# cakarsubasi/02562_raytracer

Measured on AMD Instinct MI355X. Metric: Mrays/sec primary+shadow at 1920x1080; achieved HBM GB/s vs peak, higher is better.
Workload: dtype f32

## Files before the change

02562_raytracer_amd/__init__.py:

```python
from . import _ffi
from ._ffi import MODES, TRAVERSALS, RtError, lib
from .core import (BspTree, Bvh, Context, DeviceBuffer, Mesh, empty_mask_host, load_texture_rgba8, local_tiles,
                   make_uniform)
from .render_state import ASSETS, RenderState
from .camera import CameraController
from .scenes import Camera, SceneDescriptor, find_scene, get_scenes

__all__ = ["BspTree", "Bvh", "Camera", "CameraController", "Context", "DeviceBuffer", "Mesh", "RenderState", "RtError",
           "SceneDescriptor", "ASSETS", "MODES", "TRAVERSALS", "find_scene", "get_scenes", "lib", "local_tiles",
           "load_texture_rgba8",
           "make_uniform", "_ffi"]
```

02562_raytracer_amd/_ffi.py:

```python
import ctypes as C
import os

import numpy as np

PKG_DIR = os.path.dirname(os.path.abspath(__file__))
LIB_PATH = os.environ.get("RT_LIBRARY") or os.path.join(PKG_DIR, "lib02562rt.so")

RT_OK = 0
RT_E_INVALID = -1
RT_E_OOM = -2
RT_E_DEVICE = -3
RT_E_NOT_READY = -4
RT_E_IO = -5
RT_E_UNSUPPORTED = -6

(RT_MODE_W1E6, RT_MODE_W6E1, RT_MODE_PROJECT, RT_MODE_W7E3, RT_MODE_W9E1, RT_MODE_W8E1, RT_MODE_W8E2, RT_MODE_W8E3,
 RT_MODE_W9E2, RT_MODE_W6E2, RT_MODE_W7E1, RT_MODE_W7E2, RT_MODE_W6E3, RT_MODE_W9E3,
 RT_MODE_W5E2, RT_MODE_W5E3, RT_MODE_W5E4, RT_MODE_W5E5,
 RT_MODE_W2E1, RT_MODE_W2E2, RT_MODE_W2E3, RT_MODE_W2E4, RT_MODE_W2E5,
 RT_MODE_W3E1, RT_MODE_W3E2, RT_MODE_W3E3, RT_MODE_W3E4,
 RT_MODE_W1E2, RT_MODE_W1E3, RT_MODE_W1E4, RT_MODE_W1E5) = range(31)
RT_TRAVERSE_BSP, RT_TRAVERSE_BVH, RT_TRAVERSE_NONE = range(3)
RT_OPT_DETAIL_COUNTERS = 1
RT_OPT_WAVES_PER_CU = 2
RT_OPT_SHADE_THRESHOLD = 3
RT_OPT_SAMPLE_CHUNK = 4
RT_OPT_SAMPLE_BUDGET_MB = 5
RT_OPT_UNIT_ORDER = 6
RT_OPT_BSP_CULL = 9
RT_OPT_ASYNC_FOLD = 10
RT_OPT_EMPTY_PIXELS = 11
RT_BSP_CULL_OFF, RT_BSP_CULL_CERTIFIED, RT_BSP_CULL_FAST, RT_BSP_CULL_SILHOUETTE, RT_BSP_CULL_AUTO = range(5)
BSP_TREELET_BYTES = 96
RT_OPT_KERNEL_TIMING = 7
RT_COMM_ID_BYTES = 128

MODES = {"W1E6": RT_MODE_W1E6, "W6E1": RT_MODE_W6E1, "PROJECT": RT_MODE_PROJECT, "W7E3": RT_MODE_W7E3,
         "W9E1": RT_MODE_W9E1, "W8E1": RT_MODE_W8E1, "W8E2": RT_MODE_W8E2, "W8E3": RT_MODE_W8E3,
         "W9E2": RT_MODE_W9E2, "W6E2": RT_MODE_W6E2, "W7E1": RT_MODE_W7E1, "W7E2": RT_MODE_W7E2,
         "W6E3": RT_MODE_W6E3, "W9E3": RT_MODE_W9E3,
         "W5E2": RT_MODE_W5E2, "W5E3": RT_MODE_W5E3, "W5E4": RT_MODE_W5E4, "W5E5": RT_MODE_W5E5,
         "W2E1": RT_MODE_W2E1, "W2E2": RT_MODE_W2E2, "W2E3": RT_MODE_W2E3, "W2E4": RT_MODE_W2E4,
         "W2E5": RT_MODE_W2E5, "W3E1": RT_MODE_W3E1, "W3E2": RT_MODE_W3E2, "W3E3": RT_MODE_W3E3,
         "W3E4": RT_MODE_W3E4,
         "W1E2": RT_MODE_W1E2, "W1E3": RT_MODE_W1E3, "W1E4": RT_MODE_W1E4, "W1E5": RT_MODE_W1E5}
SWEEP_MODES = ("W5E2", "W5E3", "W5E4", "W5E5")
# ... 143 lines not shown
    "rt_comm_unique_id": (C.c_int, [vp]),
    "rt_comm_init": (C.c_int, [vp, C.c_uint32, C.c_uint32, vp]),
    "rt_comm_destroy": (C.c_int, [vp]),
    "rt_gather_tiles": (C.c_int, [vp, C.c_uint32, C.c_uint32, vp, vp, vp, vp]),
    "rt_trace_rays": (C.c_int, [vp, C.c_int, vp, vp, C.c_uint32, vp]),
    "rt_trace_batch": (C.c_int, [vp, C.c_int, vp, vp, C.c_uint32, vp]),
    "rt_set_ray_capture": (C.c_int, [vp, vp, vp, C.c_uint64]),
    "rt_ray_capture_count": (C.c_int, [vp, C.POINTER(C.c_uint64)]),
    "rt_last_counts": (C.c_int, [vp, C.POINTER(RayCounts)]),
    "rt_last_elided_shadows": (C.c_int, [vp, C.POINTER(C.c_uint64)]),
    "rt_last_elided_primaries": (C.c_int, [vp, C.POINTER(C.c_uint64)]),
    "rt_empty_pixels_in_use": (C.c_int, [vp, C.POINTER(C.c_uint64), f32p]),
    "rt_empty_mask_host": (C.c_int, [f32p, C.c_uint32, u32p, C.c_uint32, C.POINTER(Uniform), u32p,
                                     C.POINTER(C.c_uint64)]),
    "rt_download_empty_mask": (C.c_int, [vp, u32p, C.c_uint64]),
    "rt_selftest_math": (C.c_int, [vp, C.c_uint32, C.c_float, C.c_float, u32p]),
    "rt_mesh_load_obj": (C.c_int, [C.c_char_p, C.POINTER(vp)]),
    "rt_mesh_from_arrays": (C.c_int, [f32p, f32p, C.c_uint32, u32p, C.c_uint32, C.POINTER(Material), C.c_uint32,
                                      C.POINTER(vp)]),
    "rt_mesh_synth_bunny": (C.c_int, [C.c_uint32, C.c_uint32, C.POINTER(vp)]),
    "rt_mesh_synth_soup": (C.c_int, [C.c_uint32, C.c_uint32, C.POINTER(vp)]),
    "rt_mesh_synth_grid": (C.c_int, [vp, C.c_uint32, C.c_uint32, C.c_float, C.POINTER(vp)]),
    "rt_mesh_scale": (C.c_int, [vp, C.c_float]),
    "rt_mesh_view_get": (C.c_int, [vp, C.POINTER(MeshView)]),
    "rt_mesh_free": (None, [vp]),
    "rt_bsp_build": (C.c_int, [vp, C.c_uint32, C.c_uint32, C.c_int, C.POINTER(vp)]),
    "rt_bsp_view_get": (C.c_int, [vp, C.POINTER(BspView)]),
    "rt_bsp_free": (None, [vp]),
    "rt_bvh_build": (C.c_int, [vp, C.c_uint32, C.POINTER(vp)]),
    "rt_bvh_view_get": (C.c_int, [vp, C.POINTER(BvhView)]),
# ... 53 lines not shown
```

02562_raytracer_amd/core.py:

```python
import ctypes as C

import numpy as np

from . import _ffi as F


def _mats_from(ptr, n):
    if n == 0:
        return np.zeros((0, 16), dtype=np.float32)
    raw = np.ctypeslib.as_array(C.cast(ptr, F.f32p), shape=(n * 16,)).copy()
    return raw.reshape(n, 16)


class Mesh:

    def __init__(self, handle):
        self._h = C.c_void_p(handle) if not isinstance(handle, C.c_void_p) else handle

    def __del__(self):
        if getattr(self, "_h", None) and self._h.value and F._lib is not None:
            F._lib.rt_mesh_free(self._h)
            self._h = C.c_void_p(None)

    @property
# ... 436 lines not shown
        n = C.c_uint64()
        self._chk(F.lib().rt_last_elided_primaries(self._h, C.byref(n)))
        return n.value

    def empty_pixels_in_use(self):
        n = C.c_uint64()
        ms = C.c_float()
        self._chk(F.lib().rt_empty_pixels_in_use(self._h, C.byref(n), C.byref(ms)))
        return n.value, ms.value

    def download_empty_mask(self, width, height):
        words = np.zeros((width * height + 31) // 32, np.uint32)
        self._chk(F.lib().rt_download_empty_mask(self._h, F.as_u32p(words), words.size))
        return _mask_bits(words, width, height)

    def timer_start(self):
        self._chk(F.lib().rt_timer_start(self._h))

    def timer_stop(self):
        ms = C.c_float()
        self._chk(F.lib().rt_timer_stop(self._h, C.byref(ms)))
        return ms.value

    def frame_rgba8(self, accum_ptr, npix, out_ptr, mode=None):
        if mode is None:
            self._chk(F.lib().rt_frame_rgba8(self._h, C.c_void_p(accum_ptr), npix, C.c_void_p(out_ptr)))
        else:
            self._chk(F.lib().rt_frame_rgba8_mode(self._h, F.MODES.get(mode, mode), C.c_void_p(accum_ptr), npix,
                                                  C.c_void_p(out_ptr)))

# ... 32 lines not shown
def _mask_bits(words, width, height):
    bits = np.unpackbits(words.view(np.uint8), bitorder="little")[:width * height]
    return bits.reshape(height, width).astype(bool)


def empty_mask_host(mesh, uniform):
    V, _, I, _, _ = mesh.arrays()
    V = np.ascontiguousarray(V, np.float32)
    I = np.ascontiguousarray(I, np.uint32)
    W, H = int(uniform.resolution[0]), int(uniform.resolution[1])
    words = np.zeros((W * H + 31) // 32, np.uint32)
    n = C.c_uint64()
    F.check(F.lib().rt_empty_mask_host(F.as_f32p(V), V.shape[0], F.as_u32p(I), I.shape[0], C.byref(uniform),
                                       F.as_u32p(words), C.byref(n)))
    return _mask_bits(words, W, H)


def load_texture_rgba8(path):
    from PIL import Image
    with Image.open(path) as im:
        return np.asarray(im.convert("RGBA"), dtype=np.uint8).copy()


def synth_texture(size=64):
    y, x = np.meshgrid(np.arange(size, dtype=np.uint32), np.arange(size, dtype=np.uint32), indexing="ij")
    h = (x * np.uint32(73856093)) ^ (y * np.uint32(19349663))
    h = (h ^ (h >> np.uint32(13))) * np.uint32(0x5BD1E995)
    h = h ^ (h >> np.uint32(15))
    t = np.empty((size, size, 4), np.uint8)
    t[..., 0] = 40 + (h & np.uint32(63))
# ... 9 lines not shown
```

02562_raytracer_amd/csrc/rt_api.cpp:

```cpp
#include <dlfcn.h>
#include <hip/hip_runtime.h>
#include <rccl/rccl.h>
#include <stdint.h>
#include <string.h>

#include <algorithm>
#include <cfloat>
#include <cmath>
#include <string>
#include <thread>
#include <type_traits>
#include <vector>

#include "host_types.h"
#include "rt_internal.h"

namespace {

struct DevBuf {
    void* p = nullptr;
    size_t n = 0;
    ~DevBuf() { reset(); }
    void reset()
    {
// ... 108 lines not shown
    bool fold_pending = false;
    float* cap_rays = nullptr;
    uint32_t* cap_flags = nullptr;
    uint64_t cap_max = 0;
    DevBuf cap_count;
    rt_noise_state* noise = nullptr;
    DevBuf noise_sum;
    uint32_t empty_opt = 1;
    float mesh_scale = 0.0f;
    float empty_cam[16] = {};
    bool empty_has_cam = false, empty_valid = false, empty_tried = false;
    uint64_t empty_iters = 0, empty_flagged = 0;
    float empty_build_ms = 0.0f;
    hipEvent_t empty_ev[2] = {nullptr, nullptr};
    DevBuf empty_mask, empty_hit, empty_cnt, empty_big;
    DevBuf act_list, act_flags, act_offs, act_scan;
    uint32_t act_key[8] = {};
    uint32_t act_n = 0, act_flagged = 0;
    bool act_valid = false;
    bool empty_used = false;
    uint64_t elided_primaries = 0;
    ncclComm_t comm = nullptr;
    uint32_t comm_nranks = 0, comm_rank = 0;
    DevBuf gather_accum, gather_ids;
};

namespace {

int fail(rt_ctx* c, int code, const std::string& msg)
{
// ... 208 lines not shown
    case RT_OPT_ASYNC_FOLD:
        if (value < 0 || value > 1) return fail(c, RT_E_INVALID, "async fold must be 0 or 1");
        if (int r = set_dev(c)) return r;
        if (value && !c->fold_stream) {
            HIPCHK(c, hipStreamCreateWithFlags(&c->fold_stream, hipStreamNonBlocking));
            for (hipEvent_t* e : {&c->ev_path, &c->ev_enter, &c->ev_fold, &c->ev_free[0], &c->ev_free[1]})
                HIPCHK(c, hipEventCreateWithFlags(e, hipEventDisableTiming));
        }
        c->async_fold = value != 0;
        return RT_OK;
    case RT_OPT_EMPTY_PIXELS:
        if (value < 0 || value > 2)
            return fail(c, RT_E_INVALID, "empty pixels must be 0 (off), 1 (on) or 2 (on, built at the first render)");
        c->empty_opt = (uint32_t)value;
        return RT_OK;
    case RT_OPT_SAMPLE_BUDGET_MB:
        if (value < 1 || value > (1 << 20)) return fail(c, RT_E_INVALID, "sample budget must be in [1,2^20] MiB");
        c->sample_budget_mb = (uint64_t)value;
        return RT_OK;
    default:
        return fail(c, RT_E_INVALID, "unknown option");
    }
}

const char* rt_last_error(const rt_ctx* c) { return c ? c->err.c_str() : rthost::get_error(); }

int rt_device_alloc(rt_ctx* c, size_t bytes, void** dptr)
{
    if (!c || !dptr) return RT_E_INVALID;
    if (int r = set_dev(c)) return r;
// ... 814 lines not shown
        unsigned long long* area_d = c->empty_cnt.as<unsigned long long>();
        uint32_t* flagged_d = c->empty_cnt.as<uint32_t>() + 2;
        uint32_t* nbig_d = c->empty_cnt.as<uint32_t>() + 3;
        HIPCHK(c, c->empty_big.ensure((size_t)std::max<uint32_t>(c->ntris, 1u) * 4));
        if (rtk::launch_empty_area(c->pos.as<float4>(), c->idx.as<uint4>(), c->nverts, c->ntris, cam14, W, H,
                                   c->mesh_scale, area_d, c->empty_big.as<uint32_t>(), nbig_d, c->stream))
            return fail(c, RT_E_DEVICE, "empty-pixel mask: launch failed");
        unsigned long long area = 0;
        uint32_t nbig = 0;
        HIPCHK(c, hipMemcpyAsync(&area, area_d, 8, hipMemcpyDeviceToHost, c->stream));
        HIPCHK(c, hipMemcpyAsync(&nbig, nbig_d, 4, hipMemcpyDeviceToHost, c->stream));
        HIPCHK(c, hipStreamSynchronize(c->stream));
        if (area <= kEmptyBudgetPerPixel * npix) {
            HIPCHK(c, c->empty_hit.ensure(npix));
            HIPCHK(c, c->empty_mask.ensure((npix + 31) / 32 * 4));
            for (hipEvent_t& e : c->empty_ev)
                if (!e) HIPCHK(c, hipEventCreate(&e));
            HIPCHK(c, hipEventRecord(c->empty_ev[0], c->stream));
            if (rtk::launch_empty_mask(c->pos.as<float4>(), c->idx.as<uint4>(), c->nverts, c->ntris, cam14, W, H,
                                       c->mesh_scale, c->empty_big.as<uint32_t>(), std::min(nbig, c->ntris),
                                       c->empty_hit.as<uint8_t>(), c->empty_mask.as<uint32_t>(), flagged_d, c->stream))
                return fail(c, RT_E_DEVICE, "empty-pixel mask: launch failed");
            HIPCHK(c, hipEventRecord(c->empty_ev[1], c->stream));
            uint32_t flagged = 0;
            HIPCHK(c, hipMemcpyAsync(&flagged, flagged_d, 4, hipMemcpyDeviceToHost, c->stream));
            HIPCHK(c, hipStreamSynchronize(c->stream));
            HIPCHK(c, hipEventElapsedTime(&c->empty_build_ms, c->empty_ev[0], c->empty_ev[1]));
            c->empty_flagged = flagged;
            c->empty_valid = true;
            c->act_valid = false;
            if (!c->auto_cull) c->probe_n = 0;
        }
    }
    *use = c->empty_valid && c->empty_flagged > 0;
    return RT_OK;
}
// ... 112 lines not shown
    L.work_counter = c->work.as<uint32_t>();
    L.cap_rays = reinterpret_cast<float4*>(c->cap_rays);
    L.cap_flags = c->cap_flags;
    L.cap_count = c->cap_count.as<unsigned long long>();
    L.cap_max = c->cap_max;
    if (trav == RT_TRAVERSE_BVH) {
        const size_t need = rtk::bvh_deep_bytes(c->num_cus, c->waves_per_cu);
        if (c->bvh_deep.n < need) HIPCHK(c, c->bvh_deep.alloc(need));
        L.bvh_deep = c->bvh_deep.as<uint32_t>();
    }
    const bool sil = has_silhouette(c, mode, trav);
    S.bsp_cull_mode = cull_in_use(c, sil);
    L.shade_threshold = default_threshold(c, mode, trav, S.bsp_cull_mode);
    L.counters = c->counters.as<unsigned long long>();
    HIPCHK(c, hipMemsetAsync(c->counters.p, 0, 32 * sizeof(unsigned long long), c->stream));
    c->empty_used = false;
    c->elided_primaries = 0;
    if (L.nwork == 0 || (L.spp == 0 && (path || direct_prog))) {
        if (counts) return rt_last_counts(c, counts);
        return RT_OK;
    }
    if (path) {
        L.stride = L.tileset ? L.nwork * 64u : L.w * L.h;
        bool ep = false;
        if (empty_applies(c, mode, trav)) {
            if (int r = ensure_empty(c, L.cam, L.spp, &ep)) return r;
            if (ep)
                if (int r = ensure_active(c, L)) return r;
            if (ep) {
                c->empty_used = true;
                c->elided_primaries = (uint64_t)c->act_flagged * L.spp;
            }
        }
        const bool nothing_active = ep && L.nactive == 0;
        const uint32_t* emask = ep ? c->empty_mask.as<uint32_t>() : nullptr;
        const uint64_t per_it = (uint64_t)L.stride * sizeof(float4);
        const uint64_t budget = c->sample_budget_mb << 20;
        uint32_t pass_spp = (uint32_t)std::min<uint64_t>(L.spp, std::max<uint64_t>(1, budget / per_it));
        const uint64_t need = per_it * pass_spp;
        const bool async = c->async_fold && c->fold_stream;
        if (c->samples.n < need) HIPCHK(c, c->samples.alloc(need));
        if (async && c->samples2.n < need) HIPCHK(c, c->samples2.alloc(need));
        L.samples = c->samples.as<float4>();
        const bool autop = sil && c->bsp_cull == RT_BSP_CULL_AUTO && c->hcam_valid && !c->detail && !nothing_active;
        if (autop)
            if (int r = probe_begin(c)) return r;
// ... 503 lines not shown
}

int rt_download_empty_mask(rt_ctx* c, uint32_t* mask_words, uint64_t nwords)
{
    if (!c || !mask_words) return RT_E_INVALID;
    memset(mask_words, 0, (size_t)nwords * 4);
    if (!c->empty_used) return RT_OK;
    if (int r = set_dev(c)) return r;
    const uint64_t have = ((uint64_t)c->u.resolution[0] * c->u.resolution[1] + 31) / 32;
    HIPCHK(c, hipMemcpyAsync(mask_words, c->empty_mask.p, (size_t)std::min(have, nwords) * 4, hipMemcpyDeviceToHost,
                             c->stream));
    HIPCHK(c, hipStreamSynchronize(c->stream));
    return RT_OK;
}

int rt_selftest_math(rt_ctx* c, uint32_t n, float lo, float hi, uint32_t* mismatches)
{
    if (!c || !mismatches || n == 0) return RT_E_INVALID;
    if (int r = set_dev(c)) return r;
    std::vector<float> in(n), hout((size_t)n * rtk::kMathOuts), dout((size_t)n * rtk::kMathOuts);
    uint32_t s = 12345u;
    for (uint32_t i = 0; i < n; i++) {
        s = s * 1664525u + 1013904223u;
        const float t = (float)i / (float)n;
        in[i] = lo + (hi - lo) * t + ((float)(s >> 8) * (1.0f / 16777216.0f) - 0.5f) * ((hi - lo) / (float)n);
    }
    rtk::host_math(in.data(), hout.data(), n);
    DevBuf din, dres;
    if (int r = upload(c, din, in.data(), in.size() * 4)) return r;
    HIPCHK(c, dres.alloc(dout.size() * 4));
// ... 38 lines not shown
```

02562_raytracer_amd/csrc/rt_empty.h:

```cpp
#pragma once
#include <stdint.h>

#if defined(__HIPCC__) || defined(__CUDACC__)
#define RT_EMPTY_HD __host__ __device__ inline
#else
#define RT_EMPTY_HD inline
#endif

namespace rtempty {

constexpr double U24 = 0x1p-24;
constexpr double SQRT3_UP = 1.7320508075688774;
constexpr double UP = 1.0 + 1e-6, DN = 1.0 - 1e-6;

struct Cam {
    double o[3], A[3], B[3], C[3];
    double M[9];
    double invW, invH;
    double pad;
    double scene;
    uint32_t W, H;
    uint32_t ok;
};

// ... 156 lines not shown
    double fx0 = (smin - cam.invH - cam.pad + 0.5) * W - 0.5 - 2.0;
    double fx1 = (smax + cam.pad + 0.5) * W - 0.5 + 2.0;
    double fy0 = (0.5 - cam.pad - tmax) * H - 0.5 - 2.0;
    double fy1 = (0.5 + cam.invH + cam.pad - tmin) * H - 0.5 + 2.0;
    if (!(fin(fx0) && fin(fx1) && fin(fy0) && fin(fy1))) return;
    if (fx1 < 0.0 || fy1 < 0.0 || fx0 > W - 1.0 || fy0 > H - 1.0) {
        x1 = -1;
        return;
    }
    x0 = (int32_t)mx(fx0, 0.0);
    y0 = (int32_t)mx(fy0, 0.0);
    x1 = (int32_t)mn(fx1 + 1.0, W - 1.0);
    y1 = (int32_t)mn(fy1 + 1.0, H - 1.0);
}

RT_EMPTY_HD bool may_hit(const Cam& cam, const Tri& t, uint32_t x, uint32_t y)
{
    if (t.kind != 1) return t.kind == 2;
    const double ux = ((double)x + 0.5) * cam.invW - 0.5, uy = 0.5 - ((double)y + 0.5) * cam.invH;
    const double s0 = ux - cam.pad, s1 = ux + cam.invH + cam.pad;
    const double t0 = uy - cam.pad, t1 = uy + cam.invH + cam.pad;
    const double sc = 0.5 * (s0 + s1), tc = 0.5 * (t0 + t1);
    const double hs = 0.5 * (s1 - s0) * (1.0 + 0x1p-40), ht = 0.5 * (t1 - t0) * (1.0 + 0x1p-40);
    double qc[3], r[3], qhi = 0.0, qlo = 0.0, wn = 0.0, wr = 0.0, sum1 = 0.0;
    for (int a = 0; a < 3; a++) {
        qc[a] = cam.A[a] * sc + cam.B[a] * tc + cam.C[a];
        r[a] = ab(cam.A[a]) * hs + ab(cam.B[a]) * ht;
        qhi += ab(qc[a]) + r[a];
        qlo = mx(qlo, ab(qc[a]) - r[a]);
        wn += qc[a] * t.nh[a];
        wr += r[a] * ab(t.nh[a]);
        sum1 += ab(qc[a]) + r[a];
// ... 10 lines not shown
    double q[4][3];
    for (int k = 0; k < 4; k++)
        for (int a = 0; a < 3; a++) q[k][a] = cam.A[a] * cs[k] + cam.B[a] * ct[k] + cam.C[a];
    const int pa[4] = {0, 1, 0, 2}, pb[4] = {2, 3, 1, 3};
    for (int k = 0; k < 4; k++) {
        const double* u = q[pa[k]];
        const double* v = q[pb[k]];
        double n[3] = {u[1] * v[2] - u[2] * v[1], u[2] * v[0] - u[0] * v[2], u[0] * v[1] - u[1] * v[0]};
        const double side = n[0] * qc[0] + n[1] * qc[1] + n[2] * qc[2];
        if (side == 0.0 || !fin(side)) return true;
        const double sg = side > 0.0 ? 1.0 : -1.0;
        double far = 0.0;
        for (int a = 0; a < 3; a++) far += sg * n[a] * t.c[a] + ab(n[a]) * (t.h[a] + m);
        if (far < 0.0) return false;
    }
    return true;
}

}
```

02562_raytracer_amd/csrc/rt_empty.hip:

```cpp
#include <vector>

#include "rt_device_common.h"
#include "rt_empty.h"

namespace rtk {

namespace {

struct TriRect {
    rtempty::Tri t;
    int32_t x0, x1, y0, y1;
};

__host__ __device__ inline TriRect tri_setup(const rtempty::Cam& cam, const float4* pos, const uint4* idx,
                                             uint32_t nverts, uint32_t k)
{
    TriRect r;
    const uint4 id = idx[k];
    if (id.x >= nverts || id.y >= nverts || id.z >= nverts) {
        r.t = rtempty::Tri{};
        r.t.kind = 2;
    } else {
        const float4 a = pos[id.x], b = pos[id.y], c = pos[id.z];
        const float v0[3] = {a.x, a.y, a.z}, v1[3] = {b.x, b.y, b.z}, v2[3] = {c.x, c.y, c.z};
// ... 11 lines not shown
constexpr unsigned long long kBigArea = 4096;
constexpr uint32_t kBigSplit = 32;

__global__ void __launch_bounds__(256) k_empty_area(const float4* pos, const uint4* idx, uint32_t nverts, uint32_t ntris,
                                                    rtempty::Cam cam, unsigned long long* area, uint32_t* big,
                                                    uint32_t* nbig)
{
    const uint32_t k = blockIdx.x * blockDim.x + threadIdx.x;
    unsigned long long a = 0;
    if (k < ntris) a = rect_area(tri_setup(cam, pos, idx, nverts, k));
    if (a > kBigArea) big[atomicAdd(nbig, 1u)] = k;
    for (int off = 32; off > 0; off >>= 1) a += __shfl_xor(a, off, 64);
    if ((threadIdx.x & 63u) == 0 && a) atomicAdd(area, a);
}

__global__ void __launch_bounds__(256) k_empty_mark(const float4* pos, const uint4* idx, uint32_t nverts, uint32_t ntris,
                                                    rtempty::Cam cam, uint8_t* hit)
{
    __shared__ TriRect sh;
    for (uint32_t k = blockIdx.x; k < ntris; k += gridDim.x) {
        __syncthreads();
        if (threadIdx.x == 0) sh = tri_setup(cam, pos, idx, nverts, k);
        __syncthreads();
        const int32_t x0 = sh.x0, y0 = sh.y0;
        if (sh.x1 < x0 || sh.y1 < y0) continue;
        const uint32_t rw = (uint32_t)(sh.x1 - x0 + 1), rh = (uint32_t)(sh.y1 - y0 + 1);
        const unsigned long long n = (unsigned long long)rw * rh;
        if (n > kBigArea) continue;
        for (unsigned long long i = threadIdx.x; i < n; i += blockDim.x) {
            const uint32_t ry = (uint32_t)(i / rw), rx = (uint32_t)(i - (unsigned long long)ry * rw);
            const uint32_t x = (uint32_t)x0 + rx, y = (uint32_t)y0 + ry;
            if (x < cam.W && y < cam.H && rtempty::may_hit(cam, sh.t, x, y)) hit[(size_t)y * cam.W + x] = 1;
        }
    }
}

__global__ void __launch_bounds__(256) k_empty_mark_big(const float4* pos, const uint4* idx, uint32_t nverts,
                                                        const uint32_t* big, rtempty::Cam cam, uint8_t* hit)
{
    __shared__ TriRect sh;
    if (threadIdx.x == 0) sh = tri_setup(cam, pos, idx, nverts, big[blockIdx.x]);
    __syncthreads();
    const int32_t x0 = sh.x0, y0 = sh.y0;
    if (sh.x1 < x0 || sh.y1 < y0) return;
    const uint32_t rw = (uint32_t)(sh.x1 - x0 + 1), rh = (uint32_t)(sh.y1 - y0 + 1);
    const unsigned long long n = (unsigned long long)rw * rh;
    for (unsigned long long i = (unsigned long long)blockIdx.y * blockDim.x + threadIdx.x; i < n;
         i += (unsigned long long)gridDim.y * blockDim.x) {
        const uint32_t ry = (uint32_t)(i / rw), rx = (uint32_t)(i - (unsigned long long)ry * rw);
        const uint32_t x = (uint32_t)x0 + rx, y = (uint32_t)y0 + ry;
        if (x < cam.W && y < cam.H && rtempty::may_hit(cam, sh.t, x, y)) hit[(size_t)y * cam.W + x] = 1;
    }
}

__global__ void __launch_bounds__(256) k_empty_pack(const uint8_t* hit, uint32_t npix, uint32_t* mask, uint32_t* flagged)
{
    const uint32_t nwords = (npix + 31u) / 32u;
    const uint32_t w = blockIdx.x * blockDim.x + threadIdx.x;
    uint32_t bits = 0;
    if (w < nwords) {
        for (uint32_t b = 0; b < 32u; b++) {
            const uint32_t i = w * 32u + b;
            if (i < npix && hit[i] == 0) bits |= 1u << b;
        }
        mask[w] = bits;
    }
// ... 33 lines not shown
int launch_empty_area(const float4* pos, const uint4* idx, uint32_t nverts, uint32_t ntris, const float cam14[14],
                      uint32_t W, uint32_t H, float scale, unsigned long long* area, uint32_t* big, uint32_t* nbig,
                      hipStream_t stream)
{
    if (hipMemsetAsync(area, 0, 8, stream) != hipSuccess) return RT_E_DEVICE;
    if (hipMemsetAsync(nbig, 0, 4, stream) != hipSuccess) return RT_E_DEVICE;
    if (ntris == 0) return 0;
    const rtempty::Cam cam = cam_of(cam14, W, H, scale);
    hipLaunchKernelGGL(k_empty_area, dim3((ntris + 255u) / 256u), dim3(256), 0, stream, pos, idx, nverts, ntris, cam, area,
                       big, nbig);
    return hipGetLastError() == hipSuccess ? 0 : RT_E_DEVICE;
}

int launch_empty_mask(const float4* pos, const uint4* idx, uint32_t nverts, uint32_t ntris, const float cam14[14],
                      uint32_t W, uint32_t H, float scale, const uint32_t* big, uint32_t nbig, uint8_t* hit,
                      uint32_t* mask, uint32_t* flagged, hipStream_t stream)
{
    const uint32_t npix = W * H;
    if (hipMemsetAsync(hit, 0, npix, stream) != hipSuccess) return RT_E_DEVICE;
    if (hipMemsetAsync(flagged, 0, 4, stream) != hipSuccess) return RT_E_DEVICE;
    const rtempty::Cam cam = cam_of(cam14, W, H, scale);
    if (ntris)
        hipLaunchKernelGGL(k_empty_mark, dim3(std::min<uint32_t>(ntris, 1u << 20)), dim3(256), 0, stream, pos, idx, nverts,
                           ntris, cam, hit);
    if (nbig)
        hipLaunchKernelGGL(k_empty_mark_big, dim3(nbig, kBigSplit), dim3(256), 0, stream, pos, idx, nverts, big, cam, hit);
    const uint32_t nwords = (npix + 31u) / 32u;
    hipLaunchKernelGGL(k_empty_pack, dim3((nwords + 255u) / 256u), dim3(256), 0, stream, hit, npix, mask, flagged);
    return hipGetLastError() == hipSuccess ? 0 : RT_E_DEVICE;
}

int build_active_list(const DevLaunch& l, const uint32_t* empty_mask, uint32_t* flags, uint32_t* offs, uint32_t* scan, uint32_t* active,
                      uint32_t* nactive, hipStream_t stream)
{
    const uint32_t nslots = l.nwork * 64u;
    *nactive = 0;
    if (nslots == 0) return 0;
    hipLaunchKernelGGL(k_slot_flags, dim3((nslots + 255u) / 256u), dim3(256), 0, stream, l, empty_mask, nslots, flags);
    if (hipGetLastError() != hipSuccess) return RT_E_DEVICE;
    if (int r = scan_exclusive_u32(flags, offs, nslots, scan, stream)) return r;
    hipLaunchKernelGGL(k_slot_scatter, dim3((nslots + 255u) / 256u), dim3(256), 0, stream, flags, offs, nslots, active);
    if (hipGetLastError() != hipSuccess) return RT_E_DEVICE;
    uint32_t last[2] = {0, 0};
    if (hipMemcpyAsync(&last[0], offs + (nslots - 1), 4, hipMemcpyDeviceToHost, stream) != hipSuccess) return RT_E_DEVICE;
    if (hipMemcpyAsync(&last[1], flags + (nslots - 1), 4, hipMemcpyDeviceToHost, stream) != hipSuccess) return RT_E_DEVICE;
    if (hipStreamSynchronize(stream) != hipSuccess) return RT_E_DEVICE;
    *nactive = last[0] + last[1];
    return 0;
}

}

extern "C" int rt_empty_mask_host(const float* pos_vec4, uint32_t nverts, const uint32_t* idx_vec4, uint32_t ntris,
                                  const rt_uniform* u, uint32_t* mask_words, uint64_t* flagged)
{
    if (!pos_vec4 || !idx_vec4 || !u || !mask_words) return RT_E_INVALID;
    const uint32_t W = u->resolution[0], H = u->resolution[1];
    if (W == 0 || H == 0 || W >= 65536u || H >= 65536u) return RT_E_INVALID;
    const size_t npix = (size_t)W * H, nwords = (npix + 31) / 32;
    for (size_t w = 0; w < nwords; w++) mask_words[w] = 0;
    if (flagged) *flagged = 0;
    float scale = 0.0f;
    for (size_t v = 0; v < nverts; v++)
        for (int a = 0; a < 3; a++) {
            const float x = pos_vec4[4 * v + a];
            if (x - x == 0.0f) scale = std::max(scale, x < 0 ? -x : x);
        }
    float cam14[14];
    rtk::camera_basis(*u, cam14);
    const rtempty::Cam cam = rtempty::make_cam(cam14, W, H, (double)scale);
    bool eye_ok = cam.ok != 0;
    for (int a = 0; a < 3; a++) eye_ok = eye_ok && rtempty::fin(cam.o[a]);
    if (!eye_ok || u->subdivision_level > 1u) return RT_OK;
    std::vector<uint8_t> hit(npix, 0);
    const float4* pos = reinterpret_cast<const float4*>(pos_vec4);
    const uint4* idx = reinterpret_cast<const uint4*>(idx_vec4);
    for (uint32_t k = 0; k < ntris; k++) {
        const rtk::TriRect r = rtk::tri_setup(cam, pos, idx, nverts, k);
        for (int32_t y = r.y0; y <= r.y1 && r.x0 <= r.x1; y++)
            for (int32_t x = r.x0; x <= r.x1; x++)
                if (!hit[(size_t)y * W + x] && rtempty::may_hit(cam, r.t, (uint32_t)x, (uint32_t)y)) hit[(size_t)y * W + x] = 1;
    }
    uint64_t n = 0;
    for (size_t i = 0; i < npix; i++)
        if (!hit[i]) {
            mask_words[i >> 5] |= 1u << (i & 31);
            n++;
        }
    if (flagged) *flagged = n;
    return RT_OK;
}
```

02562_raytracer_amd/csrc/rt_internal.h:

```cpp
#pragma once
#include <hip/hip_runtime.h>
#include <stdint.h>

#include <algorithm>
#include <string>
#include <type_traits>

#include "../../include/rt.h"

namespace rtk {

struct DevScene {
    const float4* pos;
    const float4* nrm;
    const uint4* tri_idx;
    const rt_material* mats;
    const uint32_t* lights;
    uint32_t nverts, ntris, nmats, nlights;
    const uint2* bsp_nodes;
    const float4* bsp_recs;
    uint32_t bsp_bytes;
    uint32_t bsp_rec_off;
    const uint32_t* bsp_ids;
    uint32_t bsp_depth;
// ... 5 lines not shown
    uint32_t bvh_nnodes;
    float bsp_cull_gap;
    float bsp_margin;
    float cull_k1, cull_k3, cull_ko;
    float cam_eye[3];
    float bsp_cull_emax;
    const uint2* bsp_tm;
    const uint4* bsp_sil;
    uint32_t bsp_cull_mode;
    uint32_t bsp_div_checked;
};

struct DevLaunch {
    rt_uniform u;
    float cam[14];
    const float* jitter;
    float env[3];
    const uint32_t* env_tex;
    uint32_t env_w, env_h;
    uint32_t tileset;
    uint32_t x0, y0, w, h;
    uint32_t rank, nranks;
    uint32_t tiles_x, tiles_y;
    uint32_t nwork;
    uint32_t first_iter, spp;
    uint32_t shade_threshold;
    uint32_t nactive;
    uint32_t chunk, nchunks;
    uint32_t unit_order;
    uint32_t stride;
    float4* samples;
// ... 111 lines not shown
                      const float4* pos, const uint4* idx, const uint32_t* ids, uint32_t nids, float margin,
                      void* box_scratch, uint2* tm, hipStream_t stream);
int scan_exclusive_u32(const uint32_t* in, uint32_t* out, uint32_t n, uint32_t* scratch, hipStream_t s);
size_t scan_scratch_words(uint32_t n);
int radix_sort_pairs(uint32_t* k0, uint32_t* v0, uint32_t* k1, uint32_t* v1, uint32_t n, uint32_t passes,
                     uint32_t* hist, hipStream_t s, int& result_in_second);
size_t radix_hist_words(uint32_t n);

int launch_selftest_math(const float* in, float* out, uint32_t n, hipStream_t stream);

int launch_empty_area(const float4* pos, const uint4* idx, uint32_t nverts, uint32_t ntris, const float cam14[14],
                      uint32_t W, uint32_t H, float scale, unsigned long long* area, uint32_t* big, uint32_t* nbig,
                      hipStream_t stream);
int launch_empty_mask(const float4* pos, const uint4* idx, uint32_t nverts, uint32_t ntris, const float cam14[14],
                      uint32_t W, uint32_t H, float scale, const uint32_t* big, uint32_t nbig, uint8_t* hit,
                      uint32_t* mask, uint32_t* flagged, hipStream_t stream);
int build_active_list(const DevLaunch& l, const uint32_t* empty_mask, uint32_t* flags, uint32_t* offs, uint32_t* scan, uint32_t* active,
                      uint32_t* nactive, hipStream_t stream);

void camera_basis(const rt_uniform& u, float cam[14]);

void host_math(const float* in, float* out, uint32_t n);

constexpr int kMathOuts = 16;

}
```

02562_raytracer_amd/csrc/rt_kernels.hip:

```cpp
#include <type_traits>
#include <hip/hip_runtime.h>
#include <stdint.h>

#include <algorithm>

#include "../../include/rt_detmath.h"
#include "rt_internal.h"
#include "rt_scene3.h"

namespace rtk {

__device__ __forceinline__ uint32_t lane_v()
{
    uint32_t l;
    asm volatile("v_mbcnt_lo_u32_b32 %0, -1, 0\n\tv_mbcnt_hi_u32_b32 %0, -1, %0" : "=v"(l));
    return l;
}

__device__ __forceinline__ float qmax(float a, float b)
{
    float r;
    asm("v_max_f32 %0, %1, %2" : "=v"(r) : "v"(a), "v"(b));
    return r;
}
// ... 930 lines not shown
        float jx = rnd(rng);
        float jy = rnd(rng);
        jx = jx / fH;
        jy = jy / fH;
        float ux, uy;
        pixel_uv(u, px, py, ux, uy);
        rd = cam_dir(cam, ux, uy, jx, jy);
        ro = cam.e;
        res = V(0, 0, 0);
        fac = V(1, 1, 1);
        emit = true;
        bounce = 0;
        prim = 0xFFFFFFFFu;
        shadow = false;
        inv = trav_inv<TRAV>(rd);
        trav_start<TRAV>(tr, stk, ETA, ray_tmax<MODE>(ro, rd, ETA));
        capture_ray<COUNT>(L, ro, rd, ETA, ray_tmax<MODE>(ro, rd, ETA), false);
        st = ST_TRACE;
        ao = false;
        hph = 0;
        cnt.v[C_SAMPLES]++;
        cnt.v[C_PRIMARY]++;
    };

#ifndef RT_THI_SHARE_NUM
#define RT_THI_SHARE_NUM 1
#define RT_THI_SHARE_DEN 2
#endif
    int32_t leaf_score = 0;
    uint64_t tstamp = COUNT ? __builtin_amdgcn_s_memtime() : 0;
    for (;;) {
// ... 1170 lines not shown
```

include/rt.h:

```cpp
#ifndef RT02562_RT_H
#define RT02562_RT_H

#include <stddef.h>
#include <stdint.h>

#ifdef __cplusplus
extern "C" {
#endif

#define RT_ABI_VERSION 1

#define RT_OK            0
#define RT_E_INVALID    (-1)
#define RT_E_OOM        (-2)
#define RT_E_DEVICE     (-3)
#define RT_E_NOT_READY  (-4)
#define RT_E_IO         (-5)
#define RT_E_UNSUPPORTED (-6)


typedef struct rt_material {
    float diffuse[4];
    float ambient[4];
    float specular[4];
// ... 103 lines not shown
#define RT_OPT_DETAIL_COUNTERS 1
#define RT_OPT_WAVES_PER_CU    2
#define RT_OPT_SHADE_THRESHOLD 3
#define RT_OPT_SAMPLE_CHUNK    4
#define RT_OPT_SAMPLE_BUDGET_MB 5
#define RT_OPT_KERNEL_TIMING   7
#define RT_OPT_UNIT_ORDER      6
#define RT_OPT_ASYNC_FOLD     10
#define RT_OPT_BSP_CULL        9
#define RT_BSP_CULL_OFF        0
#define RT_BSP_CULL_CERTIFIED  1
#define RT_BSP_CULL_FAST       2
#define RT_BSP_CULL_SILHOUETTE 3
#define RT_BSP_CULL_AUTO       4
#define RT_OPT_EMPTY_PIXELS   11


typedef struct rt_ctx rt_ctx;

int rt_device_count(int* count);

int rt_create(int device, rt_ctx** out);
void rt_destroy(rt_ctx* ctx);

int rt_set_stream(rt_ctx* ctx, void* hip_stream);
void* rt_get_stream(rt_ctx* ctx);
int rt_synchronize(rt_ctx* ctx);

int rt_set_option(rt_ctx* ctx, int option, int64_t value);

int rt_bsp_cull_in_use(rt_ctx* ctx, int* mode, float* probe_ms, uint32_t* probes);

int rt_empty_pixels_in_use(rt_ctx* ctx, uint64_t* pixels_flagged, float* build_ms);

int rt_empty_mask_host(const float* pos_vec4, uint32_t nverts, const uint32_t* idx_vec4, uint32_t ntris,
                       const rt_uniform* u, uint32_t* mask_words, uint64_t* flagged);
int rt_download_empty_mask(rt_ctx* ctx, uint32_t* mask_words, uint64_t nwords);
const char* rt_last_error(const rt_ctx* ctx);

int rt_device_alloc(rt_ctx* ctx, size_t bytes, void** dptr);
int rt_device_free(rt_ctx* ctx, void* dptr);
int rt_memcpy_to_host(rt_ctx* ctx, void* dst, const void* src_dev, size_t bytes);
int rt_memcpy_to_device(rt_ctx* ctx, void* dst_dev, const void* src, size_t bytes);
int rt_memset_device(rt_ctx* ctx, void* dst_dev, int value, size_t bytes);

int rt_timer_start(rt_ctx* ctx);
int rt_timer_stop(rt_ctx* ctx, float* ms);

int rt_kernel_time(rt_ctx* ctx, int reset, double* total_ms, uint32_t* launches);

int rt_gather_time(rt_ctx* ctx, int reset, double* transfer_ms, double* unpack_ms, uint32_t* calls);

// ... 187 lines not shown
```

Baseline: 15170.

## Clip primary ray interval with conservative per-pixel depth bounds from empty-pixel raster

The empty-pixel rasterization pass now also computes conservative near/far distance bounds per pixel, using interval arithmetic over each triangle's bounding box and atomic min/max. The primary-ray traversal clamps its t interval to these bounds, so BSP/BVH traversal can skip nodes outside the range. The bounds are built once per camera alongside the existing mask. The cost is extra double-precision work and atomics in the mask build and a per-pixel load at ray start. A host reference and a download API are added for validation.

Measured after the change: 17070 (median of 6 runs). 12.6% higher.

```diff
diff --git a/02562_raytracer_amd/__init__.py b/02562_raytracer_amd/__init__.py
--- a/02562_raytracer_amd/__init__.py
+++ b/02562_raytracer_amd/__init__.py
@@ -1,7 +1,7 @@
 from . import _ffi
 from ._ffi import MODES, TRAVERSALS, RtError, lib
 from .core import (BspTree, Bvh, Context, DeviceBuffer, Mesh, empty_mask_host, load_texture_rgba8, local_tiles,
-                   make_uniform)
+                   make_uniform, pixel_depth_host)
 from .render_state import ASSETS, RenderState
 from .camera import CameraController
 from .scenes import Camera, SceneDescriptor, find_scene, get_scenes
diff --git a/02562_raytracer_amd/_ffi.py b/02562_raytracer_amd/_ffi.py
--- a/02562_raytracer_amd/_ffi.py
+++ b/02562_raytracer_amd/_ffi.py
@@ -30,6 +30,7 @@
 RT_OPT_BSP_CULL = 9
 RT_OPT_ASYNC_FOLD = 10
 RT_OPT_EMPTY_PIXELS = 11
+RT_OPT_PIXEL_DEPTH = 12
 RT_BSP_CULL_OFF, RT_BSP_CULL_CERTIFIED, RT_BSP_CULL_FAST, RT_BSP_CULL_SILHOUETTE, RT_BSP_CULL_AUTO = range(5)
 BSP_TREELET_BYTES = 96
 RT_OPT_KERNEL_TIMING = 7
@@ -203,6 +204,8 @@
     "rt_empty_mask_host": (C.c_int, [f32p, C.c_uint32, u32p, C.c_uint32, C.POINTER(Uniform), u32p,
                                      C.POINTER(C.c_uint64)]),
     "rt_download_empty_mask": (C.c_int, [vp, u32p, C.c_uint64]),
+    "rt_pixel_depth_host": (C.c_int, [f32p, C.c_uint32, u32p, C.c_uint32, C.POINTER(Uniform), f32p, f32p]),
+    "rt_last_pixel_depth": (C.c_int, [vp, f32p, f32p, C.c_uint64, C.POINTER(C.c_int)]),
     "rt_selftest_math": (C.c_int, [vp, C.c_uint32, C.c_float, C.c_float, u32p]),
     "rt_mesh_load_obj": (C.c_int, [C.c_char_p, C.POINTER(vp)]),
     "rt_mesh_from_arrays": (C.c_int, [f32p, f32p, C.c_uint32, u32p, C.c_uint32, C.POINTER(Material), C.c_uint32,
diff --git a/02562_raytracer_amd/core.py b/02562_raytracer_amd/core.py
--- a/02562_raytracer_amd/core.py
+++ b/02562_raytracer_amd/core.py
@@ -474,6 +474,13 @@
         self._chk(F.lib().rt_download_empty_mask(self._h, F.as_u32p(words), words.size))
         return _mask_bits(words, width, height)
 
+    def last_pixel_depth(self, width, height):
+        near = np.empty(width * height, np.float32)
+        far = np.empty(width * height, np.float32)
+        used = C.c_int()
+        self._chk(F.lib().rt_last_pixel_depth(self._h, F.as_f32p(near), F.as_f32p(far), near.size, C.byref(used)))
+        return near.reshape(height, width), far.reshape(height, width), bool(used.value)
+
     def timer_start(self):
         self._chk(F.lib().rt_timer_start(self._h))
 
@@ -536,6 +543,18 @@
     F.check(F.lib().rt_empty_mask_host(F.as_f32p(V), V.shape[0], F.as_u32p(I), I.shape[0], C.byref(uniform),
                                        F.as_u32p(words), C.byref(n)))
     return _mask_bits(words, W, H)
+
+
+def pixel_depth_host(mesh, uniform):
+    V, _, I, _, _ = mesh.arrays()
+    V = np.ascontiguousarray(V, np.float32)
+    I = np.ascontiguousarray(I, np.uint32)
+    W, H = int(uniform.resolution[0]), int(uniform.resolution[1])
+    near = np.empty(W * H, np.float32)
+    far = np.empty(W * H, np.float32)
+    F.check(F.lib().rt_pixel_depth_host(F.as_f32p(V), V.shape[0], F.as_u32p(I), I.shape[0], C.byref(uniform),
+                                        F.as_f32p(near), F.as_f32p(far)))
+    return near.reshape(H, W), far.reshape(H, W)
 
 
 def load_texture_rgba8(path):
diff --git a/02562_raytracer_amd/csrc/rt_api.cpp b/02562_raytracer_amd/csrc/rt_api.cpp
--- a/02562_raytracer_amd/csrc/rt_api.cpp
+++ b/02562_raytracer_amd/csrc/rt_api.cpp
@@ -146,6 +146,8 @@
     float empty_build_ms = 0.0f;
     hipEvent_t empty_ev[2] = {nullptr, nullptr};
     DevBuf empty_mask, empty_hit, empty_cnt, empty_big;
+    DevBuf empty_depth;
+    bool depth_opt = true, depth_used = false;
     DevBuf act_list, act_flags, act_offs, act_scan;
     uint32_t act_key[8] = {};
     uint32_t act_n = 0, act_flagged = 0;
@@ -384,6 +386,10 @@
             return fail(c, RT_E_INVALID, "empty pixels must be 0 (off), 1 (on) or 2 (on, built at the first render)");
         c->empty_opt = (uint32_t)value;
         return RT_OK;
+    case RT_OPT_PIXEL_DEPTH:
+        if (value < 0 || value > 1) return fail(c, RT_E_INVALID, "pixel depth must be 0 (off) or 1 (on)");
+        c->depth_opt = value != 0;
+        return RT_OK;
     case RT_OPT_SAMPLE_BUDGET_MB:
         if (value < 1 || value > (1 << 20)) return fail(c, RT_E_INVALID, "sample budget must be in [1,2^20] MiB");
         c->sample_budget_mb = (uint64_t)value;
@@ -1228,12 +1234,14 @@
         if (area <= kEmptyBudgetPerPixel * npix) {
             HIPCHK(c, c->empty_hit.ensure(npix));
             HIPCHK(c, c->empty_mask.ensure((npix + 31) / 32 * 4));
+            HIPCHK(c, c->empty_depth.ensure(npix * sizeof(uint2)));
             for (hipEvent_t& e : c->empty_ev)
                 if (!e) HIPCHK(c, hipEventCreate(&e));
             HIPCHK(c, hipEventRecord(c->empty_ev[0], c->stream));
             if (rtk::launch_empty_mask(c->pos.as<float4>(), c->idx.as<uint4>(), c->nverts, c->ntris, cam14, W, H,
                                        c->mesh_scale, c->empty_big.as<uint32_t>(), std::min(nbig, c->ntris),
-                                       c->empty_hit.as<uint8_t>(), c->empty_mask.as<uint32_t>(), flagged_d, c->stream))
+                                       c->empty_hit.as<uint8_t>(), c->empty_mask.as<uint32_t>(), flagged_d,
+                                       c->empty_depth.as<uint2>(), c->stream))
                 return fail(c, RT_E_DEVICE, "empty-pixel mask: launch failed");
             HIPCHK(c, hipEventRecord(c->empty_ev[1], c->stream));
             uint32_t flagged = 0;
@@ -1376,7 +1384,7 @@
     L.shade_threshold = default_threshold(c, mode, trav, S.bsp_cull_mode);
     L.counters = c->counters.as<unsigned long long>();
     HIPCHK(c, hipMemsetAsync(c->counters.p, 0, 32 * sizeof(unsigned long long), c->stream));
-    c->empty_used = false;
+    c->empty_used = c->depth_used = false;
     c->elided_primaries = 0;
     if (L.nwork == 0 || (L.spp == 0 && (path || direct_prog))) {
         if (counts) return rt_last_counts(c, counts);
@@ -1385,6 +1393,7 @@
     if (path) {
         L.stride = L.tileset ? L.nwork * 64u : L.w * L.h;
         bool ep = false;
+        L.pix_depth = nullptr;
         if (empty_applies(c, mode, trav)) {
             if (int r = ensure_empty(c, L.cam, L.spp, &ep)) return r;
             if (ep)
@@ -1392,6 +1401,8 @@
             if (ep) {
                 c->empty_used = true;
                 c->elided_primaries = (uint64_t)c->act_flagged * L.spp;
+                c->depth_used = c->depth_opt && c->bsp_cull != RT_BSP_CULL_OFF;
+                if (c->depth_used) L.pix_depth = c->empty_depth.as<float2>();
             }
         }
         const bool nothing_active = ep && L.nactive == 0;
@@ -1925,6 +1936,27 @@
     return RT_OK;
 }
 
+int rt_last_pixel_depth(rt_ctx* c, float* near_out, float* far_out, uint64_t npix, int* in_use)
+{
+    if (!c || !near_out || !far_out) return RT_E_INVALID;
+    if (in_use) *in_use = c->depth_used ? 1 : 0;
+    for (uint64_t i = 0; i < npix; i++) {
+        near_out[i] = 0.0f;
+        far_out[i] = INFINITY;
+    }
+    if (!c->depth_used) return RT_OK;
+    if (int r = set_dev(c)) return r;
+    const uint64_t have = std::min<uint64_t>((uint64_t)c->u.resolution[0] * c->u.resolution[1], npix);
+    std::vector<float> pairs((size_t)have * 2);
+    HIPCHK(c, hipMemcpyAsync(pairs.data(), c->empty_depth.p, pairs.size() * 4, hipMemcpyDeviceToHost, c->stream));
+    HIPCHK(c, hipStreamSynchronize(c->stream));
+    for (uint64_t i = 0; i < have; i++) {
+        near_out[i] = pairs[2 * i];
+        far_out[i] = pairs[2 * i + 1];
+    }
+    return RT_OK;
+}
+
 int rt_selftest_math(rt_ctx* c, uint32_t n, float lo, float hi, uint32_t* mismatches)
 {
     if (!c || !mismatches || n == 0) return RT_E_INVALID;
diff --git a/02562_raytracer_amd/csrc/rt_empty.h b/02562_raytracer_amd/csrc/rt_empty.h
--- a/02562_raytracer_amd/csrc/rt_empty.h
+++ b/02562_raytracer_amd/csrc/rt_empty.h
@@ -194,8 +194,13 @@
     y1 = (int32_t)mn(fy1 + 1.0, H - 1.0);
 }
 
-RT_EMPTY_HD bool may_hit(const Cam& cam, const Tri& t, uint32_t x, uint32_t y)
-{
+RT_EMPTY_HD void pair_depth(const Cam& cam, const Tri& t, const double qc[3], const double r[3], double m, double depth[2]);
+RT_EMPTY_HD bool may_hit(const Cam& cam, const Tri& t, uint32_t x, uint32_t y, double* depth = nullptr)
+{
+    if (depth) {
+        depth[0] = 0.0;
+        depth[1] = __builtin_huge_val();
+    }
     if (t.kind != 1) return t.kind == 2;
     const double ux = ((double)x + 0.5) * cam.invW - 0.5, uy = 0.5 - ((double)y + 0.5) * cam.invH;
     const double s0 = ux - cam.pad, s1 = ux + cam.invH + cam.pad;
@@ -236,7 +241,80 @@
         for (int a = 0; a < 3; a++) far += sg * n[a] * t.c[a] + ab(n[a]) * (t.h[a] + m);
         if (far < 0.0) return false;
     }
+    if (depth) pair_depth(cam, t, qc, r, m, depth);
     return true;
 }
 
-}
+RT_EMPTY_HD void sqrt_bounds(double x, double& lo, double& hi)
+{
+    lo = hi = 0.0;
+    if (!(x > 0.0)) return;
+    double z = x, s = 1.0;
+    for (int k = 0; k < 540 && z >= 4.0; k++) {
+        z *= 0.25;
+        s *= 2.0;
+    }
+    for (int k = 0; k < 540 && z < 0.25; k++) {
+        z *= 4.0;
+        s *= 0.5;
+    }
+    double y = 0.5 * (1.0 + z);
+    for (int k = 0; k < 6; k++) y = 0.5 * (y + z / y);
+    hi = y * s * (1.0 + 0x1p-48);
+    lo = x / hi * (1.0 - 0x1p-48);
+}
+
+RT_EMPTY_HD void pair_depth(const Cam& cam, const Tri& t, const double qc[3], const double r[3], double m, double depth[2])
+{
+    const double up = 1.0 + 0x1p-40, dn = 1.0 - 0x1p-40;
+    double q2lo = 0.0, q2hi = 0.0, d2lo = 0.0, d2hi = 0.0, xl[3], xh[3];
+    for (int a = 0; a < 3; a++) {
+        const double ql = mx(ab(qc[a]) - r[a], 0.0), qh = ab(qc[a]) + r[a];
+        q2lo += ql * ql;
+        q2hi += qh * qh;
+        const double H = (t.h[a] + m + cam.scene * 0x1p-40) * up;
+        xl[a] = t.c[a] - H;
+        xh[a] = t.c[a] + H;
+        const double dl = mx(ab(t.c[a]) - H, 0.0), dh = ab(t.c[a]) + H;
+        d2lo += dl * dl;
+        d2hi += dh * dh;
+    }
+    if (!fin(q2hi) || !fin(d2hi) || !(q2lo > 0.0)) return;
+    double nlo, nhi, blo, bhi, tmp;
+    sqrt_bounds(q2lo * dn, nlo, tmp);
+    sqrt_bounds(q2hi * up, tmp, nhi);
+    sqrt_bounds(d2lo * dn, blo, tmp);
+    sqrt_bounds(d2hi * up, tmp, bhi);
+    if (!(nlo > 0.0) || !fin(nhi) || !fin(bhi)) return;
+    double lo = blo / UP * dn, hi = bhi / DN * up;
+    for (int a = 0; a < 3; a++) {
+        double ql = qc[a] - r[a], qh = qc[a] + r[a], al = xl[a], ah = xh[a];
+        if (qh < 0.0) {
+            const double q0 = ql, a0 = al;
+            ql = -qh;
+            qh = -q0;
+            al = -ah;
+            ah = -a0;
+        }
+        if (!(ql > 0.0) || !(ah > 0.0)) continue;
+        const double wl = ql / nhi * DN * dn, wh = qh / nlo * UP * up;
+        if (!(wl > 0.0) || !fin(wh)) continue;
+        hi = mn(hi, ah / wl * up);
+        if (al > 0.0) lo = mx(lo, al / wh * dn);
+    }
+    lo *= 1.0 - 0x1p-19;
+    hi *= 1.0 + 0x1p-19;
+    if (!(lo >= 0x1p-100)) lo = 0.0;
+    if (hi != hi) return;
+    if (!(hi >= 0x1p-100)) hi = 0x1p-100;
+    depth[0] = lo;
+    depth[1] = hi;
+}
+
+RT_EMPTY_HD void depth_f32(const double depth[2], float& nearf, float& farf)
+{
+    nearf = (float)depth[0];
+    farf = depth[1] < 3.0e38 ? (float)depth[1] : __builtin_huge_valf();
+}
+
+}
diff --git a/02562_raytracer_amd/csrc/rt_empty.hip b/02562_raytracer_amd/csrc/rt_empty.hip
--- a/02562_raytracer_amd/csrc/rt_empty.hip
+++ b/02562_raytracer_amd/csrc/rt_empty.hip
@@ -49,8 +49,27 @@
     if ((threadIdx.x & 63u) == 0 && a) atomicAdd(area, a);
 }
 
+__device__ __forceinline__ void mark_pixel(const rtempty::Cam& cam, const rtempty::Tri& t, uint32_t x, uint32_t y,
+                                           uint8_t* hit, uint2* depth)
+{
+    double d[2];
+    if (!rtempty::may_hit(cam, t, x, y, d)) return;
+    const size_t i = (size_t)y * cam.W + x;
+    hit[i] = 1;
+    float nf, ff;
+    rtempty::depth_f32(d, nf, ff);
+    atomicMin(&depth[i].x, __float_as_uint(nf));
+    atomicMax(&depth[i].y, __float_as_uint(ff));
+}
+
+__global__ void __launch_bounds__(256) k_depth_init(uint2* depth, uint32_t npix)
+{
+    const uint32_t i = blockIdx.x * blockDim.x + threadIdx.x;
+    if (i < npix) depth[i] = make_uint2(0x7F800000u, 0u);
+}
+
 __global__ void __launch_bounds__(256) k_empty_mark(const float4* pos, const uint4* idx, uint32_t nverts, uint32_t ntris,
-                                                    rtempty::Cam cam, uint8_t* hit)
+                                                    rtempty::Cam cam, uint8_t* hit, uint2* depth)
 {
     __shared__ TriRect sh;
     for (uint32_t k = blockIdx.x; k < ntris; k += gridDim.x) {
@@ -65,13 +84,14 @@
         for (unsigned long long i = threadIdx.x; i < n; i += blockDim.x) {
             const uint32_t ry = (uint32_t)(i / rw), rx = (uint32_t)(i - (unsigned long long)ry * rw);
             const uint32_t x = (uint32_t)x0 + rx, y = (uint32_t)y0 + ry;
-            if (x < cam.W && y < cam.H && rtempty::may_hit(cam, sh.t, x, y)) hit[(size_t)y * cam.W + x] = 1;
+            if (x < cam.W && y < cam.H) mark_pixel(cam, sh.t, x, y, hit, depth);
         }
     }
 }
 
 __global__ void __launch_bounds__(256) k_empty_mark_big(const float4* pos, const uint4* idx, uint32_t nverts,
-                                                        const uint32_t* big, rtempty::Cam cam, uint8_t* hit)
+                                                        const uint32_t* big, rtempty::Cam cam, uint8_t* hit,
+                                                        uint2* depth)
 {
     __shared__ TriRect sh;
     if (threadIdx.x == 0) sh = tri_setup(cam, pos, idx, nverts, big[blockIdx.x]);
@@ -84,7 +104,7 @@
          i += (unsigned long long)gridDim.y * blockDim.x) {
         const uint32_t ry = (uint32_t)(i / rw), rx = (uint32_t)(i - (unsigned long long)ry * rw);
         const uint32_t x = (uint32_t)x0 + rx, y = (uint32_t)y0 + ry;
-        if (x < cam.W && y < cam.H && rtempty::may_hit(cam, sh.t, x, y)) hit[(size_t)y * cam.W + x] = 1;
+        if (x < cam.W && y < cam.H) mark_pixel(cam, sh.t, x, y, hit, depth);
     }
 }
 
@@ -148,17 +168,19 @@
 
 int launch_empty_mask(const float4* pos, const uint4* idx, uint32_t nverts, uint32_t ntris, const float cam14[14],
                       uint32_t W, uint32_t H, float scale, const uint32_t* big, uint32_t nbig, uint8_t* hit,
-                      uint32_t* mask, uint32_t* flagged, hipStream_t stream)
+                      uint32_t* mask, uint32_t* flagged, uint2* depth, hipStream_t stream)
 {
     const uint32_t npix = W * H;
     if (hipMemsetAsync(hit, 0, npix, stream) != hipSuccess) return RT_E_DEVICE;
+    hipLaunchKernelGGL(k_depth_init, dim3((npix + 255u) / 256u), dim3(256), 0, stream, depth, npix);
     if (hipMemsetAsync(flagged, 0, 4, stream) != hipSuccess) return RT_E_DEVICE;
     const rtempty::Cam cam = cam_of(cam14, W, H, scale);
     if (ntris)
         hipLaunchKernelGGL(k_empty_mark, dim3(std::min<uint32_t>(ntris, 1u << 20)), dim3(256), 0, stream, pos, idx, nverts,
-                           ntris, cam, hit);
+                           ntris, cam, hit, depth);
     if (nbig)
-        hipLaunchKernelGGL(k_empty_mark_big, dim3(nbig, kBigSplit), dim3(256), 0, stream, pos, idx, nverts, big, cam, hit);
+        hipLaunchKernelGGL(k_empty_mark_big, dim3(nbig, kBigSplit), dim3(256), 0, stream, pos, idx, nverts, big, cam, hit,
+                           depth);
     const uint32_t nwords = (npix + 31u) / 32u;
     hipLaunchKernelGGL(k_empty_pack, dim3((nwords + 255u) / 256u), dim3(256), 0, stream, hit, npix, mask, flagged);
     return hipGetLastError() == hipSuccess ? 0 : RT_E_DEVICE;
@@ -185,6 +207,22 @@
 
 }
 
+static bool host_cam(const float* pos_vec4, uint32_t nverts, const rt_uniform& u, rtempty::Cam& cam)
+{
+    float scale = 0.0f;
+    for (size_t v = 0; v < nverts; v++)
+        for (int a = 0; a < 3; a++) {
+            const float x = pos_vec4[4 * v + a];
+            if (x - x == 0.0f) scale = std::max(scale, x < 0 ? -x : x);
+        }
+    float cam14[14];
+    rtk::camera_basis(u, cam14);
+    cam = rtempty::make_cam(cam14, u.resolution[0], u.resolution[1], (double)scale);
+    bool eye_ok = cam.ok != 0;
+    for (int a = 0; a < 3; a++) eye_ok = eye_ok && rtempty::fin(cam.o[a]);
+    return eye_ok;
+}
+
 extern "C" int rt_empty_mask_host(const float* pos_vec4, uint32_t nverts, const uint32_t* idx_vec4, uint32_t ntris,
                                   const rt_uniform* u, uint32_t* mask_words, uint64_t* flagged)
 {
@@ -194,17 +232,8 @@
     const size_t npix = (size_t)W * H, nwords = (npix + 31) / 32;
     for (size_t w = 0; w < nwords; w++) mask_words[w] = 0;
     if (flagged) *flagged = 0;
-    float scale = 0.0f;
-    for (size_t v = 0; v < nverts; v++)
-        for (int a = 0; a < 3; a++) {
-            const float x = pos_vec4[4 * v + a];
-            if (x - x == 0.0f) scale = std::max(scale, x < 0 ? -x : x);
-        }
-    float cam14[14];
-    rtk::camera_basis(*u, cam14);
-    const rtempty::Cam cam = rtempty::make_cam(cam14, W, H, (double)scale);
-    bool eye_ok = cam.ok != 0;
-    for (int a = 0; a < 3; a++) eye_ok = eye_ok && rtempty::fin(cam.o[a]);
+    rtempty::Cam cam;
+    const bool eye_ok = host_cam(pos_vec4, nverts, *u, cam);
     if (!eye_ok || u->subdivision_level > 1u) return RT_OK;
     std::vector<uint8_t> hit(npix, 0);
     const float4* pos = reinterpret_cast<const float4*>(pos_vec4);
@@ -224,3 +253,41 @@
     if (flagged) *flagged = n;
     return RT_OK;
 }
+
+extern "C" int rt_pixel_depth_host(const float* pos_vec4, uint32_t nverts, const uint32_t* idx_vec4, uint32_t ntris,
+                                   const rt_uniform* u, float* near_out, float* far_out)
+{
+    if (!pos_vec4 || !idx_vec4 || !u || !near_out || !far_out) return RT_E_INVALID;
+    const uint32_t W = u->resolution[0], H = u->resolution[1];
+    if (W == 0 || H == 0 || W >= 65536u || H >= 65536u) return RT_E_INVALID;
+    const size_t npix = (size_t)W * H;
+    rtempty::Cam cam;
+    const bool eye_ok = host_cam(pos_vec4, nverts, *u, cam);
+    if (!eye_ok || u->subdivision_level > 1u) {
+        for (size_t i = 0; i < npix; i++) {
+            near_out[i] = 0.0f;
+            far_out[i] = __builtin_huge_valf();
+        }
+        return RT_OK;
+    }
+    for (size_t i = 0; i < npix; i++) {
+        near_out[i] = __builtin_huge_valf();
+        far_out[i] = 0.0f;
+    }
+    const float4* pos = reinterpret_cast<const float4*>(pos_vec4);
+    const uint4* idx = reinterpret_cast<const uint4*>(idx_vec4);
+    for (uint32_t k = 0; k < ntris; k++) {
+        const rtk::TriRect r = rtk::tri_setup(cam, pos, idx, nverts, k);
+        for (int32_t y = r.y0; y <= r.y1 && r.x0 <= r.x1; y++)
+            for (int32_t x = r.x0; x <= r.x1; x++) {
+                double d[2];
+                if (!rtempty::may_hit(cam, r.t, (uint32_t)x, (uint32_t)y, d)) continue;
+                float nf, ff;
+                rtempty::depth_f32(d, nf, ff);
+                const size_t i = (size_t)y * W + x;
+                near_out[i] = std::min(near_out[i], nf);
+                far_out[i] = std::max(far_out[i], ff);
+            }
+    }
+    return RT_OK;
+}
diff --git a/02562_raytracer_amd/csrc/rt_internal.h b/02562_raytracer_amd/csrc/rt_internal.h
--- a/02562_raytracer_amd/csrc/rt_internal.h
+++ b/02562_raytracer_amd/csrc/rt_internal.h
@@ -43,7 +43,10 @@
 struct DevLaunch {
     rt_uniform u;
     float cam[14];
-    const float* jitter;
+    union {
+        const float* jitter;
+        const float2* pix_depth;
+    };
     float env[3];
     const uint32_t* env_tex;
     uint32_t env_w, env_h;
@@ -185,7 +188,7 @@
                       hipStream_t stream);
 int launch_empty_mask(const float4* pos, const uint4* idx, uint32_t nverts, uint32_t ntris, const float cam14[14],
                       uint32_t W, uint32_t H, float scale, const uint32_t* big, uint32_t nbig, uint8_t* hit,
-                      uint32_t* mask, uint32_t* flagged, hipStream_t stream);
+                      uint32_t* mask, uint32_t* flagged, uint2* depth, hipStream_t stream);
 int build_active_list(const DevLaunch& l, const uint32_t* empty_mask, uint32_t* flags, uint32_t* offs, uint32_t* scan, uint32_t* active,
                       uint32_t* nactive, hipStream_t stream);
 
diff --git a/02562_raytracer_amd/csrc/rt_kernels.hip b/02562_raytracer_amd/csrc/rt_kernels.hip
--- a/02562_raytracer_amd/csrc/rt_kernels.hip
+++ b/02562_raytracer_amd/csrc/rt_kernels.hip
@@ -968,7 +968,15 @@
         prim = 0xFFFFFFFFu;
         shadow = false;
         inv = trav_inv<TRAV>(rd);
-        trav_start<TRAV>(tr, stk, ETA, ray_tmax<MODE>(ro, rd, ETA));
+        float t0 = ETA, t1 = ray_tmax<MODE>(ro, rd, ETA);
+        if constexpr (EMPTYPX) {
+            if (L.pix_depth) {
+                const float2 nf = L.pix_depth[py * u.resolution[0] + px];
+                t0 = fmaxf(t0, nf.x);
+                t1 = fminf(t1, nf.y);
+            }
+        }
+        trav_start<TRAV>(tr, stk, t0, t1);
         capture_ray<COUNT>(L, ro, rd, ETA, ray_tmax<MODE>(ro, rd, ETA), false);
         st = ST_TRACE;
         ao = false;
diff --git a/include/rt.h b/include/rt.h
--- a/include/rt.h
+++ b/include/rt.h
@@ -141,6 +141,7 @@
 #define RT_BSP_CULL_SILHOUETTE 3
 #define RT_BSP_CULL_AUTO       4
 #define RT_OPT_EMPTY_PIXELS   11
+#define RT_OPT_PIXEL_DEPTH    12
 
 
 typedef struct rt_ctx rt_ctx;
@@ -163,6 +164,9 @@
 int rt_empty_mask_host(const float* pos_vec4, uint32_t nverts, const uint32_t* idx_vec4, uint32_t ntris,
                        const rt_uniform* u, uint32_t* mask_words, uint64_t* flagged);
 int rt_download_empty_mask(rt_ctx* ctx, uint32_t* mask_words, uint64_t nwords);
+int rt_pixel_depth_host(const float* pos_vec4, uint32_t nverts, const uint32_t* idx_vec4, uint32_t ntris,
+                        const rt_uniform* u, float* near_out, float* far_out);
+int rt_last_pixel_depth(rt_ctx* ctx, float* near_out, float* far_out, uint64_t npix, int* in_use);
 const char* rt_last_error(const rt_ctx* ctx);
 
 int rt_device_alloc(rt_ctx* ctx, size_t bytes, void** dptr);
```
